# zhong-yy/volpick

Hardware: AMD Instinct MI355X
Metric: waveform-windows/sec (higher is better)
Workload: dtype f32 (exact 3xbf16 split products, fp32 accumulate)

## Files before the change

### volpick_amd/csrc/eqt_mid_parts.h

```cpp
#pragma once
#include "eqt_kernels.h"
#include "prepost.h"
#include "conv_valu.h"
#if !defined(MID_TID) || !defined(MID_NT) || !defined(MID_TEAM)
#error "define MID_TID / MID_NT / MID_TEAM before including eqt_mid_parts.h"
#endif

__device__ __forceinline__ bool team_vote_or(bool mine) {
  const int team = __builtin_amdgcn_readfirstlane(MID_TEAM);
  return __builtin_amdgcn_readfirstlane((__ockl_wgred_or_i32(mine ? (1 << team) : 0) >> team) & 1) != 0;
}

namespace vp {

namespace {

constexpr int T = EQT_T;

__device__ inline float lane_bcast(float v, int lane) {
  return __int_as_float(__builtin_amdgcn_readlane(__float_as_int(v), lane));
}
__device__ inline float rcp_fast(float x) { return __builtin_amdgcn_rcpf(x); }
__device__ inline float sigmoid_fast(float x) { return rcp_fast(1.f + __expf(-x)); }
__device__ inline float tanh_fast(float z) {
  const float t = __expf(2.f * z);
  return 1.f - 2.f * rcp_fast(t + 1.f);
}

__device__ inline int lstm_row(int lane) { return (lane & 3) * 16 + (lane >> 2); }
template <int SEL>
__device__ inline float quad_bcast(float v) {
  const int x = __float_as_int(v);
  return __int_as_float(__builtin_amdgcn_update_dpp(x, x, SEL * 0x55, 0xF, 0xF, false));
}

template <int CIN>
__device__ void lstm_project(const float* xs, float* gx, const LstmWeights w, const int t0, const int tstep) {
  const int lane = MID_TID & 63, row = lstm_row(lane);
  float wih[CIN];
#pragma unroll
  for (int c = 0; c < CIN; ++c) wih[c] = w.w_ih[row * CIN + c];
  const float b = w.b[row];
  for (int t = t0; t < T; t += tstep) {
    float a0 = b, a1 = 0.f, a2 = 0.f, a3 = 0.f;
#pragma unroll
    for (int c = 0; c < CIN; c += 4) {
      const float4 x = *reinterpret_cast<const float4*>(xs + t * CIN + c);
      a0 = fmaf(wih[c], x.x, a0);
      a1 = fmaf(wih[c + 1], x.y, a1);
      a2 = fmaf(wih[c + 2], x.z, a2);
      a3 = fmaf(wih[c + 3], x.w, a3);
    }
    gx[t * 64 + lane] = (a0 + a1) + (a2 + a3);
  }
}

__device__ inline void lstm_load_whh(f32x2 (&whh)[EQT_H / 2], const LstmWeights w) {
  const int row = lstm_row(MID_TID & 63);
  const f32x2* p = reinterpret_cast<const f32x2*>(w.w_hh + row * EQT_H);
#pragma unroll
  for (int j = 0; j < EQT_H / 2; ++j) whh[j] = p[j];
}
__device__ __forceinline__ float lstm_gate_scale(const int gate) { return gate == 2 ? -2.885390082f : -1.442695041f; }
template <int GS = 64, bool SCALED = false, bool DUMP_C = false>
__device__ void lstm_recur(const float* gx, const f32x2 (&whh)[EQT_H / 2], const bool reverse, float* hout, const int hs,
                           float* cout = nullptr, const int cs = 0) {
  const int lane = MID_TID & 63;
  const bool is_g = (lane & 3) == 2;
  float h = 0.f, c = 0.f;
  float gnext = gx[(reverse ? T - 1 : 0) * GS + lane];
  for (int s = 0; s < T; ++s) {
    const int t = reverse ? T - 1 - s : s;
    f32x2 ga = {gnext, 0.f}, gb = {0.f, 0.f};
    {
      const int sn = s + 1 < T ? s + 1 : s;
      gnext = gx[(reverse ? T - 1 - sn : sn) * GS + lane];
    }
#pragma unroll
    for (int j = 0; j < EQT_H / 2; j += 2) {
      const f32x2 ha = {lane_bcast(h, 8 * j), lane_bcast(h, 8 * j + 4)};
      const f32x2 hb = {lane_bcast(h, 8 * j + 8), lane_bcast(h, 8 * j + 12)};
      ga.x = fmaf(whh[j].x, ha.x, ga.x), ga.y = fmaf(whh[j].y, ha.y, ga.y);
      gb.x = fmaf(whh[j + 1].x, hb.x, gb.x), gb.y = fmaf(whh[j + 1].y, hb.y, gb.y);
    }
    const float g0 = ga.x, g1 = ga.y, g2 = gb.x, g3 = gb.y;
    const float g = (g0 + g1) + (g2 + g3);
    if constexpr (SCALED) {
      const float sg = rcp_fast(1.f + __builtin_amdgcn_exp2f(g));
      const float act = is_g ? fmaf(sg, 2.f, -1.f) : sg;
      float cn, og;
      asm volatile(
          "s_nop 1\n\t"
          "v_mov_b32_dpp %0, %3 quad_perm:[2,2,2,2] row_mask:0xf bank_mask:0xf\n\t"
          "v_mov_b32_dpp %1, %3 quad_perm:[3,3,3,3] row_mask:0xf bank_mask:0xf\n\t"
          "v_mul_f32_dpp %0, %3, %0 quad_perm:[0,0,0,0] row_mask:0xf bank_mask:0xf\n\t"
          "v_fmac_f32_dpp %0, %3, %2 quad_perm:[1,1,1,1] row_mask:0xf bank_mask:0xf"
          : "=&v"(cn), "=&v"(og)
          : "v"(c), "v"(act));
      c = cn;
      h = og * fmaf(rcp_fast(__builtin_amdgcn_exp2f(c * 2.885390082f) + 1.f), -2.f, 1.f);
    } else {
      const float sg = sigmoid_fast(is_g ? 2.f * g : g);
      const float act = is_g ? 2.f * sg - 1.f : sg;
      const float ig = quad_bcast<0>(act), fg = quad_bcast<1>(act), gg = quad_bcast<2>(act), og = quad_bcast<3>(act);
      c = fmaf(fg, c, ig * gg);
      h = og * tanh_fast(c);
    }
    if ((lane & 3) == 0) hout[(lane >> 2) * hs + t] = h;
    if constexpr (DUMP_C) {
      if ((lane & 3) == 0) cout[(lane >> 2) * cs + t] = c;
    }
  }
}

template <int CIN>
__device__ void lstm_direction(const float* xs, float* gx, const LstmWeights w, const bool reverse, float* hout,
                               const int hs) {
  f32x2 whh[EQT_H / 2];
  lstm_load_whh(whh, w);
  lstm_project<CIN>(xs, gx, w, 0, 1);
  lstm_recur(gx, whh, reverse, hout, hs);
}

template <int KS>
__device__ __forceinline__ void mfma_load_a(float (&a)[KS], const float* w, const int row_stride) {
  static_assert(KS % 4 == 0, "16-byte loads");
  const int lane = MID_TID & 63;
  const float4* p = reinterpret_cast<const float4*>(w + (lane & 15) * row_stride + (lane >> 4) * KS);
#pragma unroll
  for (int i = 0; i < KS / 4; ++i) {
    const float4 v = p[i];
    a[4 * i] = v.x, a[4 * i + 1] = v.y, a[4 * i + 2] = v.z, a[4 * i + 3] = v.w;
  }
}
template <int KS>
__device__ __forceinline__ void mfma_load_a_t(float (&a)[KS], const float* w, const int k_stride) {
  const int lane = MID_TID & 63;
#pragma unroll
  for (int ks = 0; ks < KS; ++ks) a[ks] = w[(lane & 15) + ((lane >> 4) * KS + ks) * k_stride];
}
__device__ __forceinline__ void load4(float (&v)[4], const float* p) {
  const float4 q = *reinterpret_cast<const float4*>(p);
  v[0] = q.x, v[1] = q.y, v[2] = q.z, v[3] = q.w;
}
template <int KS>
__device__ __forceinline__ f32x4 mfma_tile(const float (&a)[KS], const float* b, const int bs, const int n0, f32x4 acc) {
  const int lane = MID_TID & 63;
  const float* bp = b + (lane >> 4) * KS * bs + n0 + (lane & 15);
#pragma unroll
  for (int ks = 0; ks < KS; ++ks) acc = __builtin_amdgcn_mfma_f32_16x16x4f32(a[ks], bp[ks * bs], acc, 0, 0, 0);
  return acc;
}

constexpr int GXS = 65;
template <int CIN>
struct ProjFrag {
  float a[CIN / 4];
  float bias[4];
};
template <int CIN>
__device__ __forceinline__ void lstm_project_load(ProjFrag<CIN>& f, const LstmWeights w, const int q) {
  const int lane = MID_TID & 63;
  mfma_load_a<CIN / 4>(f.a, w.w_ih + q * 16 * CIN, CIN);
  load4(f.bias, w.b + q * 16 + 4 * (lane >> 4));
}
template <int CIN>
__device__ __forceinline__ void lstm_project_mfma(const ProjFrag<CIN>& f, const float* xs, float* gx, const int q) {
  const int lane = MID_TID & 63;
#pragma unroll
  for (int nt = 0; nt < 3; ++nt) {
    f32x4 acc = {f.bias[0], f.bias[1], f.bias[2], f.bias[3]};
    acc = mfma_tile<CIN / 4>(f.a, xs, 48, 16 * nt, acc);
    const int t = 16 * nt + (lane & 15);
    if (t < T) {
#pragma unroll
      for (int r = 0; r < 4; ++r) gx[t * GXS + 4 * (4 * (lane >> 4) + r) + q] = acc[r] * lstm_gate_scale(q);
    }
  }
}

constexpr int KP = 34;
__device__ __forceinline__ void attn_wa(float (&wa)[32], const float wa_lane) {
#pragma unroll
  for (int u = 0; u < 32; ++u) wa[u] = lane_bcast(wa_lane, u);
}
template <int ES, int UH = 16>
__device__ __forceinline__ void attn_scores(const float (*q)[KP], const float (*k)[KP], float* e, const float (&wa)[32], const bool plain) {
  const int tid = MID_TID, nt = MID_NT;
  if (plain) {
    for (int idx = tid; idx < T * T; idx += nt) {
      const int i = idx / T, j = idx - i * T;
      float s0 = 0.f, s1 = 0.f;
#pragma unroll
      for (int u = 0; u < 32; u += 2) {
        s0 = fmaf(wa[u], tanh_fast(q[i][u] + k[j][u]), s0);
        s1 = fmaf(wa[u + 1], tanh_fast(q[i][u + 1] + k[j][u + 1]), s1);
      }
      e[i * ES + j] = s0 + s1;
    }
  } else {
    for (int idx = tid; idx < T * T; idx += nt) {
      const int i = idx / T, j = idx - i * T;
      const f32x2* qi = reinterpret_cast<const f32x2*>(&q[i][0]);
      const f32x2* kj = reinterpret_cast<const f32x2*>(&k[j][0]);
      f32x2 s = {0.f, 0.f};
#pragma unroll
      for (int u0 = 0; u0 < 16; u0 += UH) {
        if (UH < 16 && u0 > 0) __builtin_amdgcn_sched_barrier(0);
#pragma unroll
        for (int u = u0; u < u0 + UH; ++u) {
          const f32x2 d = __builtin_elementwise_fma(qi[u], kj[u], f32x2{1.f, 1.f});
          const f32x2 r = {rcp_fast(d.x), rcp_fast(d.y)};
          s = __builtin_elementwise_fma(f32x2{wa[2 * u], wa[2 * u + 1]}, r, s);
        }
      }
      e[i * ES + j] = -2.f * (s.x + s.y);
    }
  }
}

template <int ES, bool ZERO_PAD>
__device__ __forceinline__ void attn_softmax(float* e, const float eps, const int width) {
  const int tid = MID_TID, lane = tid & 63, wave = tid >> 6, nw = MID_NT >> 6;
  constexpr int R = 3;
  const int lower = lane - width / 2;
  for (int i0 = wave; i0 < T; i0 += R * nw) {
    float x[R], m[R], ex[R], sum[R];
#pragma unroll
    for (int r = 0; r < R; ++r) {
      const int i = i0 + r * nw;
      x[r] = (lane < T && i < T) ? e[i * ES + lane] : -INFINITY;
    }
    m[0] = x[0], m[1] = x[1], m[2] = x[2];
    wave_max3(m[0], m[1], m[2]);
#pragma unroll
    for (int r = 0; r < R; ++r) {
      const int i = i0 + r * nw;
      ex[r] = (lane < T && i < T) ? __expf(x[r] - m[r]) : 0.f;
      if (width > 0 && !(lower <= i && i < lower + width)) ex[r] = 0.f;
    }
    sum[0] = ex[0], sum[1] = ex[1], sum[2] = ex[2];
    wave_sum3(sum[0], sum[1], sum[2]);
#pragma unroll
    for (int r = 0; r < R; ++r) {
      const int i = i0 + r * nw;
      if (lane < (ZERO_PAD ? T + 1 : T) && i < T) e[i * ES + lane] = ex[r] * rcp_fast(sum[r] + eps);
    }
  }
}

__device__ void attention_core(const float (*xs)[EQT_H], float (*q)[KP], float (*k)[KP], float (*e)[48],
                               float (*v)[EQT_H], const AttnWeights w, const float eps, const int width) {
  const int tid = MID_TID, nt = MID_NT;
  const float wa_lane = w.Wa[tid & 31];
  bool big = false;
  for (int idx = tid; idx < T * 32; idx += nt) {
    const int t = idx >> 5, u = idx & 31;
    float aq = 0.f, ak = w.bh[u];
#pragma unroll
    for (int c = 0; c < EQT_H; ++c) {
      aq = fmaf(xs[t][c], w.Wt[c * 32 + u], aq);
      ak = fmaf(xs[t][c], w.Wx[c * 32 + u], ak);
    }
    q[t][u] = aq;
    k[t][u] = ak;
    big |= !(fabsf(aq) <= 30.f) || !(fabsf(ak) <= 30.f);
  }
  const bool plain = team_vote_or(big);
  if (!plain) {
    for (int idx = tid; idx < T * 32; idx += nt) {
      const int t = idx >> 5, u = idx & 31;
      q[t][u] = __expf(2.f * q[t][u]);
      k[t][u] = __expf(2.f * k[t][u]);
    }
    __syncthreads();
  }
  float wa[32];
  attn_wa(wa, wa_lane);
  attn_scores<48>(q, k, &e[0][0], wa, plain);
  __syncthreads();
  attn_softmax<48, false>(&e[0][0], eps, width);
  __syncthreads();
  for (int idx = tid; idx < T * EQT_H; idx += nt) {
    const int i = idx >> 4, c = idx & 15;
    float acc = 0.f;
    const int j0 = width > 0 ? max(0, i - (width - 1 - width / 2)) : 0, j1 = width > 0 ? min(T - 1, i + width / 2) : T - 1;
    for (int j = j0; j <= j1; ++j) acc = fmaf(e[i][j], xs[j][c], acc);
    v[i][c] = acc;
  }
  __syncthreads();
}

constexpr int AES = 49;
struct AttnFrag {
  float a[4], bias[4];
};
__device__ __forceinline__ void attn_load(AttnFrag& f, const AttnWeights w) {
  const int lane = MID_TID & 63, mt = MID_TID >> 6;
  mfma_load_a_t<4>(f.a, (mt < 2 ? w.Wt : w.Wx) + 16 * (mt & 1), 32);
  load4(f.bias, w.bh + 16 * (mt & 1) + 4 * (lane >> 4));
}
struct NoPrefetch {
  __device__ void operator()() const {}
};

__device__ inline void load_window_transposed(const float* src, int ls, float (*xs)[EQT_H]) {
  for (int idx = MID_TID; idx < EQT_H * T; idx += MID_NT) {
    const int c = idx / T, t = idx - c * T;
    xs[t][c] = src[(long)c * ls + HALO + t];
  }
}

__device__ inline void layer_norm16(const float* z, const float* gamma, const float* beta, float eps, float* out) {
  float mean = 0.f;
#pragma unroll
  for (int c = 0; c < EQT_H; ++c) mean += z[c];
  mean *= (1.f / EQT_H);
  float var = 0.f;
#pragma unroll
  for (int c = 0; c < EQT_H; ++c) var = fmaf(z[c] - mean, z[c] - mean, var);
  var = var * (1.f / EQT_H) + eps;
  const float inv = 1.f / sqrtf(var);
#pragma unroll
  for (int c = 0; c < EQT_H; ++c) out[c] = (z[c] - mean) * inv * gamma[c] + beta[c];
}

template <int G0>
__device__ __forceinline__ void layer_norm_mfma(float (&z)[4], const float par, const float eps) {
  const int g = (MID_TID & 63) >> 4;
  float s = (z[0] + z[1]) + (z[2] + z[3]);
  s += __shfl_xor(s, 16);
  s += __shfl_xor(s, 32);
  const float mean = s * (1.f / EQT_H);
  float d[4], v = 0.f;
#pragma unroll
  for (int r = 0; r < 4; ++r) d[r] = z[r] - mean, v = fmaf(d[r], d[r], v);
  v += __shfl_xor(v, 16);
  v += __shfl_xor(v, 32);
  const float inv = 1.f / sqrtf(v * (1.f / EQT_H) + eps);
#pragma unroll
  for (int r = 0; r < 4; ++r) z[r] = d[r] * inv * __shfl(par, G0 + 4 * g + r) + __shfl(par, G0 + 16 + 4 * g + r);
}

}
}
```

Measured before the change: 3.585 million.

## Restructure attention softmax so each quad of lanes owns one row

Softmax is re-mapped so four lanes share one row, each covering 16 columns, and a wave handles 16 rows at once. The old scheme used one lane per column with full-wave max and sum reductions. Row reductions now happen mostly inside registers, followed by two DPP quad exchanges, which replaces the 64-lane cross-wave shuffles. The cost is more registers per lane and strided per-lane LDS accesses, which may cause bank conflicts.

Measured after the change: 3.573 million. No clear change (-0.3%).

```diff
diff --git a/volpick_amd/csrc/eqt_mid_parts.h b/volpick_amd/csrc/eqt_mid_parts.h
--- a/volpick_amd/csrc/eqt_mid_parts.h
+++ b/volpick_amd/csrc/eqt_mid_parts.h
@@ -219,32 +219,50 @@
   }
 }
 
+template <int X>
+__device__ __forceinline__ float quad_xor(const float v) {
+  static_assert(X == 1 || X == 2, "within the quad");
+  const int x = __float_as_int(v);
+  return __int_as_float(__builtin_amdgcn_update_dpp(x, x, X == 1 ? 0xB1 : 0x4E, 0xF, 0xF, false));
+}
+
 template <int ES, bool ZERO_PAD>
 __device__ __forceinline__ void attn_softmax(float* e, const float eps, const int width) {
   const int tid = MID_TID, lane = tid & 63, wave = tid >> 6, nw = MID_NT >> 6;
-  constexpr int R = 3;
-  const int lower = lane - width / 2;
-  for (int i0 = wave; i0 < T; i0 += R * nw) {
-    float x[R], m[R], ex[R], sum[R];
-#pragma unroll
-    for (int r = 0; r < R; ++r) {
-      const int i = i0 + r * nw;
-      x[r] = (lane < T && i < T) ? e[i * ES + lane] : -INFINITY;
-    }
-    m[0] = x[0], m[1] = x[1], m[2] = x[2];
-    wave_max3(m[0], m[1], m[2]);
-#pragma unroll
-    for (int r = 0; r < R; ++r) {
-      const int i = i0 + r * nw;
-      ex[r] = (lane < T && i < T) ? __expf(x[r] - m[r]) : 0.f;
-      if (width > 0 && !(lower <= i && i < lower + width)) ex[r] = 0.f;
-    }
-    sum[0] = ex[0], sum[1] = ex[1], sum[2] = ex[2];
-    wave_sum3(sum[0], sum[1], sum[2]);
-#pragma unroll
-    for (int r = 0; r < R; ++r) {
-      const int i = i0 + r * nw;
-      if (lane < (ZERO_PAD ? T + 1 : T) && i < T) e[i * ES + lane] = ex[r] * rcp_fast(sum[r] + eps);
+  constexpr int NC = 16;
+  static_assert(3 * NC == T + 1, "three quarters cover the row and its padding column");
+  const int j0 = NC * (lane & 3);
+  for (int i0 = 16 * wave; i0 < T; i0 += 16 * nw) {
+    const int i = i0 + (lane >> 2);
+    float* row = e + (i < T ? i : T - 1) * ES + j0;
+    float x[NC];
+#pragma unroll
+    for (int c = 0; c < NC; ++c) x[c] = j0 + c < T ? row[c] : -INFINITY;
+    float m = x[0];
+#pragma unroll
+    for (int c = 1; c < NC; ++c) m = fmaxf(m, x[c]);
+    m = fmaxf(m, quad_xor<1>(m));
+    m = fmaxf(m, quad_xor<2>(m));
+    const unsigned d = width > 0 ? (unsigned)(i - j0 + width / 2) : 0x40000000u, bound = width > 0 ? (unsigned)width : 0x7fffffffu;
+#pragma unroll
+    for (int c = 0; c < NC; ++c) x[c] = (j0 + c < T && d - c < bound) ? __expf(x[c] - m) : 0.f;
+    float s[NC];
+#pragma unroll
+    for (int c = 0; c < NC; ++c) s[c] = x[c];
+#pragma unroll
+    for (int w = 1; w < NC; w *= 2) {
+#pragma unroll
+      for (int c = 0; c < NC; c += 2 * w) s[c] += s[c + w];
+    }
+    float sum = s[0];
+    sum += quad_xor<1>(sum);
+    sum += quad_xor<2>(sum);
+    const float inv = rcp_fast(sum + eps);
+    if (i < T) {
+#pragma unroll
+      for (int c = 0; c < NC; ++c) {
+        if (j0 + c < (ZERO_PAD ? T + 1 : T)) row[c] = x[c] * inv;
+      }
     }
   }
 }
```
